# JackWoo0831/Yolov7-tracker

Measured on AMD Instinct MI355X. Metric: end-to-end fps (detect+track) YOLOv7-w6@1280 ByteTrack, higher is better.
Workload: dtype f16

## Files before the change

### yolov7-tracker_amd/csrc/y7t_conv_common.h

```cpp
#pragma once
#include "y7t_det.h"
#include <type_traits>

typedef _Float16 half_t;
typedef __attribute__((ext_vector_type(8))) _Float16 half8;
typedef __attribute__((ext_vector_type(4))) _Float16 half4;
typedef __attribute__((ext_vector_type(16))) float floatx16;

#define GLOBAL_AS __attribute__((address_space(1)))
#define LDS_AS __attribute__((address_space(3)))

template <int ACT>
__device__ __forceinline__ float act_t(float v) {
    if (ACT == Y7T_ACT_SILU) return v * __builtin_amdgcn_rcpf(1.0f + __builtin_amdgcn_exp2f(-1.44269504088896f * v));
    if (ACT == Y7T_ACT_LEAKY) return v > 0.f ? v : 0.1f * v;
    return v;
}

template <typename F>
__device__ __forceinline__ void act_dispatch(int act, F&& body) {
    if (act == Y7T_ACT_SILU) body(std::integral_constant<int, Y7T_ACT_SILU>{});
    else if (act == Y7T_ACT_LEAKY) body(std::integral_constant<int, Y7T_ACT_LEAKY>{});
    else body(std::integral_constant<int, Y7T_ACT_NONE>{});
}

__device__ __forceinline__ float act_fn(float v, int act) {
    if (act == Y7T_ACT_SILU) return v * __builtin_amdgcn_rcpf(1.0f + __builtin_amdgcn_exp2f(-1.44269504088896f * v));
    if (act == Y7T_ACT_LEAKY) return v > 0.f ? v : 0.1f * v;
    return v;
}
```

### yolov7-tracker_amd/csrc/y7t_conv_patch.hip

```cpp
#include "y7t_common.h"
#include "y7t_conv_common.h"
#include <stdlib.h>

namespace {

constexpr unsigned kOOB = 0xFF000000u;

template <int TW, int TH, int BN>
struct PatchCfg {
    static constexpr int PIXB = 80;
    static constexpr bool FLAT = (TW == 0);
    static constexpr int PW = TH;
    static constexpr int NPOS = 256 + 2 * PW + 2;
    static constexpr int RP = FLAT ? PW * PIXB : (TW == 16) ? 1536 : (TW + 2) * PIXB;
    static constexpr int PATCH_DMA = FLAT ? (NPOS * PIXB + 1023) / 1024 : ((TH + 2) * RP + 1023) / 1024;
    static constexpr int NPX = (PATCH_DMA + 1) / 2;
    static constexpr int PATCH_BYTES = PATCH_DMA * 1024;
    static constexpr int PPT = (NPX + 6) / 7;
    static constexpr int WROWB = 64;
    static constexpr int W_DMA = BN * WROWB / 1024;
    static constexpr int NWX = W_DMA / 2;
    static constexpr int W_BYTES = W_DMA * 1024;
    static constexpr int NWS = 3;
    static constexpr int W_OFF = 0, P_OFF = NWS * W_BYTES;
    static constexpr int LDS_LOOP = P_OFF + 2 * PATCH_BYTES;
    static constexpr int OROW = BN * 2 + 16;
    static constexpr int LDS_EPI = 256 * OROW;
    static constexpr int BIAS_OFF = LDS_LOOP > LDS_EPI + 1024 ? LDS_LOOP : LDS_EPI + 1024;
    static constexpr int LDS = BIAS_OFF + BN * 4;
    static constexpr int WN = BN / 64, WM = 4 / WN;
    static constexpr int TM = 8 / WM;
    static constexpr int RPT = (TW == 16) ? 2 : 1;
    static constexpr int JOFF = FLAT ? 32 * PIXB : RPT * RP;
};

#define Y7T_PATCH_ISSUE_DMAS() \
            { \
                constexpr bool live = !(ABL & 1); \
                if (wrole) { \
                    const int un = u + 3; \
                    const int ccn = (un / 9), tn = un % 9; \
                    const int cn = c0 + ccn; \
                    if (ABL & 16) issue_w(u % 3, 0, 0, 0, true); \
                    else issue_w(u % 3, ccn == 2 ? cbase + s_pair : cbase + ccn * s_odd, tn / 3, tn % 3, cn < nc32 && live); \
                } else if (t < 7) { \
                _Pragma("unroll") \
                    for (int q = 0; q < C::PPT; ++q) \
                        if (t * C::PPT + q < C::NPX) issue_patch_piece(cc ^ 1, c + 1, t * C::PPT + q, c + 1 < nc32 && live && !(ABL & 32)); \
                } \
            }
template <int TW, int TH, int BN, int ABL>
__global__ void __launch_bounds__(256, 2) k_conv3x3_patch(const Y7TConvArgs p) {
#if defined(__HIP_DEVICE_COMPILE__)
    using C = PatchCfg<TW, TH, BN>;
    static_assert(C::FLAT || TW * TH == 256, "256 output pixels per workgroup");
    constexpr int PIXB = C::PIXB, RP = C::RP, TM = C::TM, RPT = C::RPT;
    constexpr bool FLAT = C::FLAT;
    extern __shared__ __attribute__((aligned(16))) char smem[];
    const int tid = threadIdx.x, lane = tid & 63, wave = __builtin_amdgcn_readfirstlane(tid >> 6);
    const int wn = (C::WN == 2) ? (wave >> 1) : 0, wm = (C::WN == 2) ? (wave & 1) : wave;
    const int l31 = lane & 31, hi32 = lane >> 5;

    int bid = blockIdx.x;
    if (p.xcd_swizzle) {
        const int nwg = gridDim.x, q = nwg >> 3, r = nwg & 7, xcd = bid & 7, idx = bid >> 3;
        bid = (xcd < r ? xcd * (q + 1) : r * (q + 1) + (xcd - r) * q) + idx;
    }
    const int n_tiles_n = p.Cout_pad / BN;
    const int tile_n = bid % n_tiles_n;
    int pt = bid / n_tiles_n;
    int b = 0, h0 = 0, w0 = 0;
    const int g0 = pt * 256;
    const int img_pos = (p.H + 2) * C::PW, strip = p.B * img_pos;
    if (!FLAT) {
        constexpr int TWd = FLAT ? 1 : TW;
        const int tiles_x = (p.W + TWd - 1) / TWd, tiles_y = (p.H + TH - 1) / TH;
        const int txi = pt % tiles_x; pt /= tiles_x;
        const int tyi = pt % tiles_y;
        b = pt / tiles_y; h0 = tyi * TH; w0 = txi * TWd;
    }
    const int n0 = tile_n * BN;

    const __amdgpu_buffer_rsrc_t xr = __builtin_amdgcn_make_buffer_rsrc((void*)p.in, 0, p.in_bytes, 0x00020000);
    const __amdgpu_buffer_rsrc_t wr = __builtin_amdgcn_make_buffer_rsrc((void*)p.w, 0, p.w_bytes, 0x00020000);

    const bool wrole = wave < 2;
    constexpr int NOFF = C::NPX > C::NWX ? C::NPX : C::NWX;
    unsigned off[NOFF];
#pragma unroll
    for (int i = 0; i < NOFF; ++i) {
        unsigned v = kOOB;
        if (wrole) {
            if (i < C::NWX) {
                const int byte = (wave * C::NWX + i) * 1024 + lane * 16;
                const int row = byte >> 6, slot = (byte >> 4) & 3;
                if (p.korder == 2) v = (unsigned)(tile_n * (p.K_pad >> 5) * C::W_BYTES + byte);
                else v = (unsigned)(((n0 + row) * p.K_pad + ((slot ^ ((row >> 2) & 3)) << 3)) * 2);
            }
        } else if (i < C::NPX) {
            int I = (wave - 2) + 2 * i;
            if (I >= C::PATCH_DMA) I = C::PATCH_DMA - 1;
            const int byte = I * 1024 + lane * 16;
            if (FLAT) {
                const int q = byte / PIXB, cs = (byte - q * PIXB) >> 4;
                const int g = g0 - C::PW - 1 + q;
                if (cs < 4 && q < C::NPOS && g >= 0 && g < strip) {
                    const int bb = g / img_pos, rem = g - bb * img_pos;
                    const int yy = rem / C::PW, xx = rem - yy * C::PW;
                    if (yy >= 1 && yy <= p.H && xx >= 1 && xx <= p.W)
                        v = (unsigned)(((((bb * p.H + yy - 1) * p.W + xx - 1) * p.ldin + p.cin_off) + cs * 8) * 2);
                }
            } else {
            const int r = byte / RP, rb = byte - r * RP;
            const int x = rb / PIXB, cs = (rb - x * PIXB) >> 4;
            const int gy = h0 + r - 1, gx = w0 + x - 1;
            const bool ok = r < TH + 2 && x < TW + 2 && cs < 4 && (unsigned)gy < (unsigned)p.H && (unsigned)gx < (unsigned)p.W;
            if (ok) v = (unsigned)(((((b * p.H + gy) * p.W + gx) * p.ldin + p.cin_off) + cs * 8) * 2);
            }
        }
        off[i] = v;
    }

    const int wsw = (l31 >> 2) & 3;
    const char* wlane0 = smem + C::W_OFF + (wn * 64 + l31) * C::WROWB + (((0 + hi32) ^ wsw) << 4);
    const char* wlane1 = smem + C::W_OFF + (wn * 64 + l31) * C::WROWB + (((2 + hi32) ^ wsw) << 4);
    const char* plane = FLAT ? smem + C::P_OFF + (wm * TM * 32 + l31) * PIXB + hi32 * 16
                             : smem + C::P_OFF + (wm * TM * RPT + (TW == 16 ? (l31 >> 4) : 0)) * RP + (TW == 16 ? (l31 & 15) : l31) * PIXB + hi32 * 16;

    const int nc32 = p.Cin >> 5;
    const int s_kh = p.korder == 2 ? 3 * C::W_BYTES : p.korder ? (p.Cin >> 6) * 3 * 128 : 3 * p.Cin * 2;
    const int s_kw = p.korder == 2 ? C::W_BYTES : p.korder ? 128 : p.Cin * 2;
    const int s_odd = p.korder == 2 ? 9 * C::W_BYTES : 64;
    const int s_pair = p.korder == 2 ? 18 * C::W_BYTES : p.korder ? 3 * 128 : 128;
    int cbase = 0;
    auto issue_w = [&](int slot, int coff, int kh, int kw, bool real) {
        const int so = kh * s_kh + kw * s_kw + coff;
#pragma unroll
        for (int i = 0; i < C::NWX; ++i)
            __builtin_amdgcn_raw_ptr_buffer_load_lds(wr, (LDS_AS void*)(smem + C::W_OFF + slot * C::W_BYTES + (wave * C::NWX + i) * 1024), 16,
                                                     real ? off[i] : kOOB, real ? so : 0, 0, 0);
    };
    auto issue_patch_piece = [&](int pb, int c, int i, bool real) {
        const int I = ((wave - 2) + 2 * i < C::PATCH_DMA) ? (wave - 2) + 2 * i : C::PATCH_DMA - 1;
        __builtin_amdgcn_raw_ptr_buffer_load_lds(xr, (LDS_AS void*)(smem + C::P_OFF + pb * C::PATCH_BYTES + I * 1024), 16,
                                                 real ? off[i] : kOOB, c << 6, 0, 0);
    };

    floatx16 acc[2][TM];
#pragma unroll
    for (int i = 0; i < 2; ++i)
#pragma unroll
        for (int j = 0; j < TM; ++j)
#pragma unroll
            for (int e = 0; e < 16; ++e) acc[i][j][e] = 0.f;

    if (tid < BN) ((float*)(smem + C::BIAS_OFF))[tid] = p.bias[n0 + tid];
    if (wrole) {
        issue_w(0, 0, 0, 0, true);
        issue_w(1, 0, 0, 1, true);
        issue_w(2, 0, 0, 2, true);
    } else {
#pragma unroll
        for (int i = 0; i < C::NPX; ++i) issue_patch_piece(0, 0, i, true);
    }

    static_assert(C::PPT * 7 >= C::NPX, "patch pieces fit into taps 0..6");
    static_assert(C::LDS <= 81920, "two workgroups per CU");
    half8 wf[2][2][2], xf[2][2][TM];
    auto read_frags = [&](int buf, int slot, int pb, int kh, int kw) {
        const char* ws0 = wlane0 + slot * C::W_BYTES;
        const char* ws1 = wlane1 + slot * C::W_BYTES;
        const char* ps = plane + pb * C::PATCH_BYTES + kh * RP + kw * PIXB;
        if (ABL & 4) {
#pragma unroll
            for (int ks = 0; ks < 2; ++ks) {
#pragma unroll
                for (int i = 0; i < 2; ++i) asm volatile("" : "=v"(wf[buf][ks][i]));
#pragma unroll
                for (int j = 0; j < TM; ++j) asm volatile("" : "=v"(xf[buf][ks][j]));
            }
            return;
        }
#pragma unroll
        for (int ks = 0; ks < 2; ++ks) {
#pragma unroll
            for (int i = 0; i < 2; ++i) wf[buf][ks][i] = *(const half8*)((ks ? ws1 : ws0) + i * 32 * C::WROWB);
#pragma unroll
            for (int j = 0; j < TM; ++j) xf[buf][ks][j] = *(const half8*)(ps + j * C::JOFF + ks * 32);
        }
    };
    auto mfma_half = [&](int buf, int ks) {
        if (ABL & 2) {
#pragma unroll
            for (int i = 0; i < 2; ++i) asm volatile("" ::"v"(wf[buf][ks][i]));
#pragma unroll
            for (int j = 0; j < TM; ++j) asm volatile("" ::"v"(xf[buf][ks][j]));
            return;
        }
        __builtin_amdgcn_s_setprio(1);
#pragma unroll
        for (int i = 0; i < 2; ++i)
#pragma unroll
            for (int j = 0; j < TM; ++j) acc[i][j] = __builtin_amdgcn_mfma_f32_32x32x16_f16(wf[buf][ks][i], xf[buf][ks][j], acc[i][j], 0, 0, 0);
        __builtin_amdgcn_s_setprio(0);
    };
    if (wrole) asm volatile("s_waitcnt vmcnt(%0)" ::"n"(2 * C::NWX) : "memory");
    else asm volatile("s_waitcnt vmcnt(0)" ::: "memory");
    __builtin_amdgcn_s_barrier();
    read_frags(0, 0, 0, 0, 0);

    for (int c0 = 0; c0 < nc32; c0 += 2) {
#pragma unroll
        for (int u = 0; u < 18; ++u) {
            const int cc = u / 9, t = u % 9;
            const int c = c0 + cc, cur = u & 1;
            if (ABL == 0) {
                const int un = u + 1, tn = un % 9, kh = tn / 3, kw = tn % 3;
                const char* ps = plane + ((un / 9) & 1) * C::PATCH_BYTES + kh * RP + kw * PIXB;
                const char* ws0 = wlane0 + (un % 3) * C::W_BYTES;
                const char* ws1 = wlane1 + (un % 3) * C::W_BYTES;
                __builtin_amdgcn_s_setprio(1);
#pragma unroll
                for (int q = 0; q < 2 * TM; ++q) {
                    const int i = q / TM, j = q % TM;
                    acc[i][j] = __builtin_amdgcn_mfma_f32_32x32x16_f16(wf[cur][0][i], xf[cur][0][j], acc[i][j], 0, 0, 0);
                    if (t < 8) xf[cur ^ 1][q / TM][q % TM] = *(const half8*)(ps + (q % TM) * C::JOFF + (q / TM) * 32);
                    __builtin_amdgcn_sched_barrier(0);
                }
                __builtin_amdgcn_s_setprio(0);
                if (t < 8) asm volatile("s_waitcnt lgkmcnt(%0)" ::"n"(2 * TM) : "memory");
                else asm volatile("s_waitcnt lgkmcnt(0)" ::: "memory");
                if (wrole) asm volatile("s_waitcnt vmcnt(%0)" ::"n"(C::NWX) : "memory");
                else if (t == 8) asm volatile("s_waitcnt vmcnt(0)" ::: "memory");
                __builtin_amdgcn_s_barrier();
                Y7T_PATCH_ISSUE_DMAS()
                __builtin_amdgcn_sched_barrier(0);
                __builtin_amdgcn_s_setprio(1);
#pragma unroll
                for (int q = 0; q < 2 * TM; ++q) {
                    const int i = q / TM, j = q % TM;
                    acc[i][j] = __builtin_amdgcn_mfma_f32_32x32x16_f16(wf[cur][1][i], xf[cur][1][j], acc[i][j], 0, 0, 0);
                    if (q < 4) wf[cur ^ 1][q >> 1][q & 1] = *(const half8*)(((q >> 1) ? ws1 : ws0) + (q & 1) * 32 * C::WROWB);
                    if (t == 8) xf[cur ^ 1][q / TM][q % TM] = *(const half8*)(ps + (q % TM) * C::JOFF + (q / TM) * 32);
                    __builtin_amdgcn_sched_barrier(0);
                }
                __builtin_amdgcn_s_setprio(0);
                continue;
            }
            mfma_half(cur, 0);
            asm volatile("s_waitcnt lgkmcnt(0)" ::: "memory");
            if (wrole) asm volatile("s_waitcnt vmcnt(%0)" ::"n"(C::NWX) : "memory");
            else if (t == 8) asm volatile("s_waitcnt vmcnt(0)" ::: "memory");
            __builtin_amdgcn_s_barrier();
            if (!(ABL & 512)) Y7T_PATCH_ISSUE_DMAS()
            {
                const int un = u + 1, tn = un % 9;
                read_frags(cur ^ 1, un % 3, (un / 9) & 1, tn / 3, tn % 3);
            }
            mfma_half(cur, 1);
            if (ABL & 512) Y7T_PATCH_ISSUE_DMAS()
        }
        cbase += s_pair;
    }

    if (ABL & 8) {
#pragma unroll
        for (int i = 0; i < 2; ++i)
#pragma unroll
            for (int j = 0; j < TM; ++j) asm volatile("" ::"v"(acc[i][j]));
        return;
    }
    constexpr int OROW = C::OROW;
    const float* lbias = (const float*)(smem + C::BIAS_OFF);
    asm volatile("s_waitcnt vmcnt(0)" ::: "memory");
    __syncthreads();
    typedef __attribute__((ext_vector_type(4))) float float4v;
    act_dispatch(p.act, [&](auto act_c) {
    constexpr int ACT = decltype(act_c)::value;
#pragma unroll
    for (int j = 0; j < TM; ++j) {
        const int pix = (wm * TM + j) * 32 + l31;
#pragma unroll
        for (int i = 0; i < 2; ++i) {
            const int nl = wn * 64 + i * 32;
#pragma unroll
            for (int gp = 0; gp < 2; ++gp) {
                unsigned w[2][2];
#pragma unroll
                for (int gg = 0; gg < 2; ++gg) {
                    const int g = gp * 2 + gg;
                    const int n = n0 + nl + 8 * g + 4 * hi32;
                    float v[4];
                    const float4v bv = *(const float4v*)(lbias + (n - n0));
#pragma unroll
                    for (int e = 0; e < 4; ++e) v[e] = act_t<ACT>(acc[i][j][g * 4 + e] + bv[e]);
                    typedef __attribute__((ext_vector_type(2))) _Float16 half2v;
                    half2v h0 = {(half_t)v[0], (half_t)v[1]}, h1 = {(half_t)v[2], (half_t)v[3]};
                    w[gg][0] = __builtin_bit_cast(unsigned, h0);
                    w[gg][1] = __builtin_bit_cast(unsigned, h1);
                }
                auto r0 = __builtin_amdgcn_permlane32_swap(w[0][0], w[1][0], false, false);
                auto r1 = __builtin_amdgcn_permlane32_swap(w[0][1], w[1][1], false, false);
                typedef __attribute__((ext_vector_type(4))) unsigned uint4v;
                uint4v pk = {r0[0], r1[0], r0[1], r1[1]};
                *(uint4v*)(smem + pix * OROW + (nl + 8 * (gp * 2 + hi32)) * 2) = pk;
            }
        }
    }
    });
    int* otab = (int*)(smem + C::LDS_EPI);
    if (FLAT) {
        const int g = g0 + tid;
        int o = -1;
        if (g < strip) {
            const int bb = g / img_pos, rem = g - bb * img_pos;
            const int yy = rem / C::PW, xx = rem - yy * C::PW;
            if (yy >= 1 && yy <= p.H && xx >= 1 && xx <= p.W) o = (bb * p.H + yy - 1) * p.W + xx - 1;
        }
        otab[tid] = o;
    }
    __syncthreads();
    {
        typedef __attribute__((ext_vector_type(4))) unsigned uint4v;
        constexpr int CPP = BN / 8;
        half_t* outp = (half_t*)p.out;
        constexpr int GRP = CPP < 8 ? CPP : 8;
        static_assert(CPP % GRP == 0, "whole groups");
#pragma unroll 1
        for (int c0 = 0; c0 < CPP; c0 += GRP) {
            uint4v v[GRP];
#pragma unroll
            for (int k = 0; k < GRP; ++k) {
                const int cidx = tid + (c0 + k) * 256, pix = cidx / CPP, ch = cidx - pix * CPP;
                v[k] = *(const uint4v*)(smem + pix * OROW + ch * 16);
            }
            __builtin_amdgcn_sched_barrier(0);
#pragma unroll
            for (int k = 0; k < GRP; ++k) {
                const int cidx = tid + (c0 + k) * 256, pix = cidx / CPP, ch = cidx - pix * CPP;
                const int n = n0 + ch * 8;
                long long opix;
                if (FLAT) opix = otab[pix];
                else {
                    constexpr int TWd = FLAT ? 1 : TW;
                    const int r = pix / TWd, x = pix - r * TWd;
                    const int gy = h0 + r, gx = w0 + x;
                    opix = (gy < p.H && gx < p.W) ? (long long)(b * p.H + gy) * p.W + gx : -1;
                }
                if (opix >= 0 && n < p.Cout) *(uint4v*)(outp + (size_t)opix * p.ldout + p.cout_off + n) = v[k];
            }
        }
    }
#endif
}

template <int TW, int TH, int MT>
__global__ void __launch_bounds__(256, 2) k_conv3x3_patch_mt(const Y7TConvArgs p) {
#if defined(__HIP_DEVICE_COMPILE__)
    constexpr int BN = 64;
    using C = PatchCfg<TW, TH, BN>;
    static_assert(!C::FLAT && TW * TH == 256, "256 output pixels per tile");
    constexpr int PIXB = C::PIXB, RP = C::RP, TM = C::TM, RPT = C::RPT;
    constexpr int NWS = 3, WD = 3;
    constexpr int P_OFF = NWS * C::W_BYTES, BIAS_OFF = P_OFF + 2 * C::PATCH_BYTES;
    extern __shared__ __attribute__((aligned(16))) char smem[];
    const int tid = threadIdx.x, lane = tid & 63, wave = __builtin_amdgcn_readfirstlane(tid >> 6);
    const int wm = wave;
    const int l31 = lane & 31, hi32 = lane >> 5;
    int bid = blockIdx.x;
    if (p.xcd_swizzle) {
        const int nwg = gridDim.x, q = nwg >> 3, r = nwg & 7, xcd = bid & 7, idx = bid >> 3;
        bid = (xcd < r ? xcd * (q + 1) : r * (q + 1) + (xcd - r) * q) + idx;
    }
    const int n_tiles_n = p.Cout_pad / BN;
    const int tile_n = bid % n_tiles_n, n0 = tile_n * BN;
    const int tiles_x = (p.W + TW - 1) / TW, tiles_y = (p.H + TH - 1) / TH, ptiles = p.B * tiles_y * tiles_x;
    const int pt_first = (bid / n_tiles_n) * MT;
    const int nt = (ptiles - pt_first) < MT ? (ptiles - pt_first) : MT;

    const __amdgpu_buffer_rsrc_t xr = __builtin_amdgcn_make_buffer_rsrc((void*)p.in, 0, p.in_bytes, 0x00020000);
    const __amdgpu_buffer_rsrc_t wr = __builtin_amdgcn_make_buffer_rsrc((void*)p.w, 0, p.w_bytes, 0x00020000);
    const bool wrole = wave < 2;

    auto patch_off = [&](int pt, unsigned (&o)[C::NPX]) {
        int q = pt;
        const int txi = q % tiles_x; q /= tiles_x;
        const int tyi = q % tiles_y, b = q / tiles_y, h0 = tyi * TH, w0 = txi * TW;
#pragma unroll
        for (int i = 0; i < C::NPX; ++i) {
            int I = (wave - 2) + 2 * i;
            if (I >= C::PATCH_DMA) I = C::PATCH_DMA - 1;
            const int byte = I * 1024 + lane * 16;
            const int r = byte / RP, rb = byte - r * RP;
            const int x = rb / PIXB, cs = (rb - x * PIXB) >> 4;
            const int gy = h0 + r - 1, gx = w0 + x - 1;
            const bool ok = pt < ptiles && r < TH + 2 && x < TW + 2 && cs < 4 && (unsigned)gy < (unsigned)p.H && (unsigned)gx < (unsigned)p.W;
            o[i] = ok ? (unsigned)(((((b * p.H + gy) * p.W + gx) * p.ldin + p.cin_off) + cs * 8) * 2) : kOOB;
        }
    };
    unsigned pc[C::NPX], pn[C::NPX], woff[C::NWX];
#pragma unroll
    for (int i = 0; i < C::NPX; ++i) pc[i] = pn[i] = kOOB;
#pragma unroll
    for (int i = 0; i < C::NWX; ++i) woff[i] = kOOB;
    if (wrole) {
#pragma unroll
        for (int i = 0; i < C::NWX; ++i) {
            const int byte = (wave * C::NWX + i) * 1024 + lane * 16;
            const int row = byte >> 6, slot = (byte >> 4) & 3;
            woff[i] = p.korder == 2 ? (unsigned)(tile_n * (p.K_pad >> 5) * C::W_BYTES + byte)
                                    : (unsigned)(((n0 + row) * p.K_pad + ((slot ^ ((row >> 2) & 3)) << 3)) * 2);
        }
    } else {
        patch_off(pt_first, pc);
        patch_off(pt_first + 1, pn);
    }
    const int wsw = (l31 >> 2) & 3;
    const char* wlane0 = smem + C::W_OFF + l31 * C::WROWB + (((0 + hi32) ^ wsw) << 4);
    const char* wlane1 = smem + C::W_OFF + l31 * C::WROWB + (((2 + hi32) ^ wsw) << 4);
    const char* plane = smem + P_OFF + (wm * TM * RPT + (TW == 16 ? (l31 >> 4) : 0)) * RP + (TW == 16 ? (l31 & 15) : l31) * PIXB + hi32 * 16;

    const int nc32 = p.Cin >> 5, total = nt * nc32;
    const int s_kh = p.korder == 2 ? 3 * C::W_BYTES : p.korder ? (p.Cin >> 6) * 3 * 128 : 3 * p.Cin * 2;
    const int s_kw = p.korder == 2 ? C::W_BYTES : p.korder ? 128 : p.Cin * 2;
    auto chunk_off = [&](int c) -> int {
// ... 88 lines not shown
        }
        ct += 2;
        if (ct == nc32) {
            int q = pt_first + tcur;
            const int txi = q % tiles_x; q /= tiles_x;
            const int tyi = q % tiles_y, b = q / tiles_y, h0 = tyi * TH, w0 = txi * TW;
            act_dispatch(p.act, [&](auto act_c) {
            constexpr int ACT = decltype(act_c)::value;
            typedef __attribute__((ext_vector_type(4))) float float4v;
#pragma unroll
            for (int j = 0; j < TM; ++j) {
                const int pix = (wm * TM + j) * 32 + l31;
                const int r = pix / TW, x = pix - r * TW;
                const int gy = h0 + r, gx = w0 + x;
                const bool okp = gy < p.H && gx < p.W;
                half_t* orow = outp + ((size_t)(b * p.H + gy) * p.W + gx) * p.ldout + p.cout_off + n0;
#pragma unroll
                for (int i = 0; i < 2; ++i) {
#pragma unroll
                    for (int gp = 0; gp < 2; ++gp) {
                        unsigned w[2][2];
#pragma unroll
                        for (int gg = 0; gg < 2; ++gg) {
                            const int g = gp * 2 + gg;
                            const int nl = i * 32 + 8 * g + 4 * hi32;
                            float v[4];
                            const float4v bv = *(const float4v*)(lbias + nl);
#pragma unroll
                            for (int e = 0; e < 4; ++e) v[e] = act_t<ACT>(acc[i][j][g * 4 + e] + bv[e]);
                            typedef __attribute__((ext_vector_type(2))) _Float16 half2v;
                            half2v h0v = {(half_t)v[0], (half_t)v[1]}, h1v = {(half_t)v[2], (half_t)v[3]};
                            w[gg][0] = __builtin_bit_cast(unsigned, h0v);
                            w[gg][1] = __builtin_bit_cast(unsigned, h1v);
                        }
                        auto r0 = __builtin_amdgcn_permlane32_swap(w[0][0], w[1][0], false, false);
                        auto r1 = __builtin_amdgcn_permlane32_swap(w[0][1], w[1][1], false, false);
                        typedef __attribute__((ext_vector_type(4))) unsigned uint4v;
                        const uint4v pk = {r0[0], r1[0], r0[1], r1[1]};
                        const int nn = i * 32 + 8 * (gp * 2 + hi32);
                        if (okp && n0 + nn < p.Cout) *(uint4v*)(orow + nn) = pk;
                    }
#pragma unroll
                    for (int e = 0; e < 16; ++e) acc[i][j][e] = 0.f;
                }
            }
            });
            ct = 0;
            ++tcur;
            if (!wrole) {
#pragma unroll
                for (int i = 0; i < C::NPX; ++i) pc[i] = pn[i];
                patch_off(pt_first + tcur + 1, pn);
            }
        }
    }
#endif
}

template <int TW, int TH, int MT>
int launch_patch_mt(const Y7TConvArgs& a, hipStream_t s) {
    using C0 = PatchCfg<TW, TH, 64>;
    constexpr int lds = 3 * C0::W_BYTES + 2 * C0::PATCH_BYTES + 64 * 4;
    static_assert(lds <= 81920, "two workgroups per CU");
    static Y7TOncePerDevice attr;
    if (int e_ = y7t_once_per_device(attr, [&]() -> int {
        Y7T_HIP_CHECK(hipFuncSetAttribute((const void*)k_conv3x3_patch_mt<TW, TH, MT>, hipFuncAttributeMaxDynamicSharedMemorySize, lds));
        return 0;
    })) return e_;
    const int ptiles = a.B * ((a.H + TH - 1) / TH) * ((a.W + TW - 1) / TW);
    hipLaunchKernelGGL((k_conv3x3_patch_mt<TW, TH, MT>), dim3(((ptiles + MT - 1) / MT) * (a.Cout_pad / 64)), dim3(256), lds, s, a);
    Y7T_LAUNCH_CHECK();
    y7t_note_kernel("patch_mt<%d,%d,%d>", TW, TH, MT);
    return 0;
}

template <int TW, int TH, int BN, int ABL = 0>
int launch_patch(const Y7TConvArgs& a, hipStream_t s) {
    using C = PatchCfg<TW, TH, BN>;
    static Y7TOncePerDevice attr;
    if (int e_ = y7t_once_per_device(attr, [&]() -> int {
        Y7T_HIP_CHECK(hipFuncSetAttribute((const void*)k_conv3x3_patch<TW, TH, BN, ABL>, hipFuncAttributeMaxDynamicSharedMemorySize, C::LDS));
        return 0;
    })) return e_;
    const int ptiles = C::FLAT ? (a.B * (a.H + 2) * C::PW + 255) / 256 : a.B * ((a.H + TH - 1) / TH) * ((a.W + (C::FLAT ? 1 : TW) - 1) / (C::FLAT ? 1 : TW));
    const int tiles = ptiles * (a.Cout_pad / BN);
    hipLaunchKernelGGL((k_conv3x3_patch<TW, TH, BN, ABL>), dim3(tiles), dim3(256), C::LDS, s, a);
    Y7T_LAUNCH_CHECK();
    if (C::FLAT) y7t_note_kernel("patch_strip<%d,%d>%s", C::PW, BN, ABL == 2048 ? " burst-reads" : "");
    else y7t_note_kernel("patch<%d,%d,%d>%s", TW, TH, BN, ABL == 2048 ? " burst-reads" : "");
    return 0;
}

}

int y7t_conv_patch_try(const Y7TConvArgs& a, hipStream_t s) {
    static int mode = -1;
    if (mode < 0) mode = y7t_exp_switch("Y7T_CONV_PATCH", 1);
    const bool eligible = a.KH == 3 && a.KW == 3 && a.stride == 1 && a.pad == 1 && a.Cin % 64 == 0 && !a.out_f32 && !(a.Cout & 7) && !(a.ldout & 7) &&
                          !(a.cout_off & 7) && a.Ho == a.H && a.Wo == a.W && a.in_bytes <= kOOB - (1u << 24) && a.w_bytes <= kOOB - (1u << 24);
    if (a.korder == 2 && (!eligible || !mode)) {
        y7t_set_error("conv: weights are in panel order (korder 2) but the layer cannot run on the patch kernel");
        return Y7T_E_ARG;
    }
    if (!mode || !eligible) return 0;
    auto eff = [&](int tw, int th) {
        const int tx = (a.W + tw - 1) / tw, ty = (a.H + th - 1) / th;
        return (double)(a.W * a.H) / ((double)tx * tw * ty * th);
    };
    const double e16 = eff(16, 16), e32 = eff(32, 8);
    const bool use16 = e16 >= e32;
    const bool wide = a.Cout_pad % 128 == 0 && !a.panel64;
    const double eflat = (a.W == 40 || a.W == 20) ? (double)(a.W * a.H) / ((a.W + 2) * (a.H + 2)) : 0.0;
    if (!a.force_patch && a.korder != 2 && (long long)a.B * a.H * a.W * (a.Cout_pad / (wide ? 128 : 64)) < 256ll * 256) return 0;
    const int abl = Y7T_ABLATE ? a.ablate : 0;
    if (eflat > (use16 ? e16 : e32) && eflat >= 0.8 && (!abl || abl == 2048)) {
        int rcf;
#if Y7T_ABLATE
        if (abl == 2048) {
            if (a.W == 40) rcf = wide ? launch_patch<0, 42, 128, 2048>(a, s) : launch_patch<0, 42, 64, 2048>(a, s);
            else rcf = wide ? launch_patch<0, 22, 128, 2048>(a, s) : launch_patch<0, 22, 64, 2048>(a, s);
        } else
#endif
        if (a.W == 40) rcf = wide ? launch_patch<0, 42, 128>(a, s) : launch_patch<0, 42, 64>(a, s);
        else rcf = wide ? launch_patch<0, 22, 128>(a, s) : launch_patch<0, 22, 64>(a, s);
        return rcf ? rcf : 1;
    }
    if (!a.force_patch && a.korder != 2 && (use16 ? e16 : e32) < 0.8) return 0;
    int rc;
#if Y7T_ABLATE
    if (abl == 2048) {
        if (use16) rc = wide ? launch_patch<16, 16, 128, 2048>(a, s) : launch_patch<16, 16, 64, 2048>(a, s);
        else rc = wide ? launch_patch<32, 8, 128, 2048>(a, s) : launch_patch<32, 8, 64, 2048>(a, s);
        return rc ? rc : 1;
    }
    if (abl && use16 && wide) {
        switch (abl) {
        case 1: return launch_patch<16, 16, 128, 1>(a, s) ? -1 : 1;
        case 2: return launch_patch<16, 16, 128, 2>(a, s) ? -1 : 1;
        case 4: return launch_patch<16, 16, 128, 4>(a, s) ? -1 : 1;
        case 8: return launch_patch<16, 16, 128, 8>(a, s) ? -1 : 1;
        case 15: return launch_patch<16, 16, 128, 15>(a, s) ? -1 : 1;
        case 16: return launch_patch<16, 16, 128, 16>(a, s) ? -1 : 1;
        case 32: return launch_patch<16, 16, 128, 32>(a, s) ? -1 : 1;
        case 48: return launch_patch<16, 16, 128, 48>(a, s) ? -1 : 1;
        default: break;
        }
    }
#endif
    static int mt = -1;
    if (mt < 0) mt = y7t_exp_switch("Y7T_CONV_PATCH_MT", 1);
    const int ptiles = a.B * ((a.H + (use16 ? 15 : 7)) / (use16 ? 16 : 8)) * ((a.W + (use16 ? 15 : 31)) / (use16 ? 16 : 32));
    if (!wide && mt && !abl && (ptiles * (a.Cout_pad / 64) >= 4 * 2048 || a.force_patch)) {
        rc = use16 ? launch_patch_mt<16, 16, 4>(a, s) : launch_patch_mt<32, 8, 4>(a, s);
        return rc ? rc : 1;
    }
    if (use16) rc = wide ? launch_patch<16, 16, 128>(a, s) : launch_patch<16, 16, 64>(a, s);
    else rc = wide ? launch_patch<32, 8, 128>(a, s) : launch_patch<32, 8, 64>(a, s);
    return rc ? rc : 1;
}
```

### yolov7-tracker_amd/detector/graph.py

```python
import math

import os

import numpy as np

from .. import _lib


def make_divisible(x, divisor):
    return math.ceil(x / divisor) * divisor


class Node:
    __slots__ = ("idx", "kind", "src", "c", "k", "s", "p", "act", "wkey", "layer", "extra", "h", "w", "home", "coff", "ld", "virt_up", "virtual")

    def __init__(self, kind, src, c, k=1, s=1, p=0, act=0, wkey=None, layer=-1, extra=None):
        self.kind, self.src, self.c, self.k, self.s, self.p, self.act, self.wkey, self.layer, self.extra = kind, list(src), c, k, s, p, act, wkey, layer, extra
        self.idx = -1
        self.h = self.w = 0
        self.home, self.coff, self.ld = None, 0, 0
        self.virt_up, self.virtual = None, False


def _act_code(a):
# ... 61 lines not shown
        elif m in ("nn.Upsample", "Upsample"):
            if args[0] not in (None, "None") or args[1] != 2 or args[2] != "nearest":
                raise NotImplementedError("Upsample%r" % (args,))
            out, c2 = add(Node("up", src, cin[0], layer=i)), cin[0]
        elif m == "Shortcut":
            if len(src) != 2 or cin[0] != cin[1]:
                raise NotImplementedError("Shortcut of %d tensors with %r channels" % (len(src), cin))
            out, c2 = add(Node("add", src, cin[0], layer=i)), cin[0]
        elif m == "DownC":
            c2 = make_divisible(args[0] * gw, 8)
            k = args[2] if len(args) > 2 else 2
            key = "model.%d." % i
            cv1 = add(Node("conv", src, cin[0], 1, 1, 0, 1, key + "cv1", i))
            cv2 = add(Node("conv", [cv1], c2 // 2, 3, k, 1, 1, key + "cv2", i))
            mp = add(Node("pool", src, cin[0], k, k, 0, layer=i))
            cv3 = add(Node("conv", [mp], c2 // 2, 1, 1, 0, 1, key + "cv3", i))
            out = add(Node("concat", [cv2, cv3], c2 // 2 * 2, layer=i))
            c2 = c2 // 2 * 2
        elif m == "SPPCSPC":
            c2 = make_divisible(args[0] * gw, 8)
            c_ = int(2 * c2 * 0.5)
            key = "model.%d." % i
            cv1 = add(Node("conv", src, c_, 1, 1, 0, 1, key + "cv1", i))
            cv3 = add(Node("conv", [cv1], c_, 3, 1, 1, 1, key + "cv3", i))
            cv4 = add(Node("conv", [cv3], c_, 1, 1, 0, 1, key + "cv4", i))
            p5 = add(Node("pool", [cv4], c_, 5, 1, 2, layer=i))
            p9 = add(Node("pool", [p5], c_, 5, 1, 2, layer=i))
            p13 = add(Node("pool", [p9], c_, 5, 1, 2, layer=i))
            cat1 = add(Node("concat", [cv4, p5, p9, p13], 4 * c_, layer=i))
            cv5 = add(Node("conv", [cat1], c_, 1, 1, 0, 1, key + "cv5", i))
            cv6 = add(Node("conv", [cv5], c_, 3, 1, 1, 1, key + "cv6", i))
            cv2 = add(Node("conv", src, c_, 1, 1, 0, 1, key + "cv2", i))
            cat2 = add(Node("concat", [cv6, cv2], 2 * c_, layer=i))
            out = add(Node("conv", [cat2], c2, 1, 1, 0, 1, key + "cv7", i))
        elif m in ("Detect", "IDetect", "IAuxDetect"):
            nl = len(anchors)
            out = add(Node("detect", src[:nl], no, layer=i, extra={"kind": m, "nl": nl, "na": na, "no": nc + 5, "cin": cin[:nl]}))
            c2 = no
        else:
            raise NotImplementedError("module %s (layer %d) is outside the yolov7 family's hot path" % (m, i))
        layer_out.append(out)
        chs.append(c2)
    return nodes, layer_out


OP_DTYPE = np.dtype([("type", "<i4"), ("in_buf", "<i4"), ("in_ld", "<i4"), ("in_coff", "<i4"), ("H", "<i4"), ("W", "<i4"), ("Cin", "<i4"),
                     ("out_buf", "<i4"), ("out_ld", "<i4"), ("out_coff", "<i4"), ("out_f32", "<i4"), ("Ho", "<i4"), ("Wo", "<i4"),
                     ("Cout", "<i4"), ("Cout_pad", "<i4"), ("KH", "<i4"), ("KW", "<i4"), ("stride", "<i4"), ("pad", "<i4"), ("K", "<i4"),
                     ("K_pad", "<i4"), ("act", "<i4"), ("korder", "<i4"), ("detect_level", "<i4"), ("w_off", "<i8"), ("bias_off", "<i8"),
                     ("up_buf", "<i4"), ("up_ld", "<i4"), ("up_coff", "<i4"), ("up_c0", "<i4"), ("up_C", "<i4"), ("pad0", "<i4")], align=False)
assert OP_DTYPE.itemsize == 136


def _rup(x, m):
    return (x + m - 1) // m * m


class Plan:
    """result of `lower`: ops (structured array), buffer table, weight layout, head description"""


def patch_panel_rows(H, W, cout, B):
    cout_pad = -(-cout // 64) * 64
    if cout_pad % 128:
        return 64
    below = int(_lib.switch("Y7T_CONV_PATCH_PANEL64_BELOW", "512"))
    return 64 if B * H * W // 256 * (cout_pad // 128) < below else 128


PATCH_MIN_PIX = 100 * 256
PATCH_MIN_PIX_SHALLOW = 50 * 256


def patch_eligible(H, W, cin, cout, k, s, p, out_ld, out_coff, out_f32, B=1 << 20):
    cout_pad = -(-cout // 64) * 64
    bn = patch_panel_rows(H, W, cout, B)
    if B * H * W * (cout_pad // bn) < int(_lib.switch("Y7T_CONV_PATCH_MIN_PIX", str(PATCH_MIN_PIX_SHALLOW if cin <= 128 else PATCH_MIN_PIX))):
        return False
    if _lib.switch("Y7T_CONV_PATCH", "1") == "0" or _lib.switch("Y7T_CONV_VARIANT", "0") != "0":
        return False
    if not (k == 3 and s == 1 and p == 1 and cin % 64 == 0 and not out_f32 and cout % 8 == 0 and out_ld % 8 == 0 and out_coff % 8 == 0):
        return False
    eff = lambda tw, th: (W * H) / float(-(-W // tw) * tw * -(-H // th) * th)
    eflat = (W * H) / float((W + 2) * (H + 2)) if W in (20, 40) else 0.0
    return max(eff(16, 16), eff(32, 8), eflat) >= 0.8


def patch_s2_eligible(cin, cout, k, s, p, out_ld, out_coff, out_f32, M_out=1 << 30):
    mode = _lib.switch("Y7T_CONV_PATCH_S2", "auto")
    if mode == "0" or _lib.switch("Y7T_CONV_VARIANT", "0") != "0":
        return False
    cout_pad = -(-cout // 64) * 64
    can = (k == 3 and s == 2 and p == 1 and cin % 64 == 0 and cout_pad % 128 == 0 and not out_f32 and cout % 8 == 0 and out_ld % 8 == 0
           and out_coff % 8 == 0)
    if mode == "1":
        return can and cout_pad >= int(_lib.switch("Y7T_CONV_PATCH_S2_MIN_COUT", "128"))
    return can and cout_pad % 256 == 0 and cin >= 128 and M_out >= 50000 and _lib.switch("Y7T_CONV_PATCH_S2_BN", "") != "128"


def ws_eligible(H, W, cin, cout, k, s, p, out_ld, out_coff, out_f32, in_ld, in_coff, B=1 << 20):
    if _lib.switch("Y7T_CONV_WS", "1") == "0" or _lib.switch("Y7T_CONV_VARIANT", "0") != "0":
        return False
    tiles = B * -(-H // 16) * -(-W // 16)
    return (k == 3 and s == 1 and p == 1 and cin == 64 and cout == 64 and H % 16 == 0 and W % 16 == 0 and not out_f32 and out_ld % 8 == 0 and out_coff % 8 == 0 and in_ld % 8 == 0
            and in_coff % 8 == 0 and tiles >= int(_lib.switch("Y7T_CONV_WS_MIN_TILES", "1024")))


def ws_s2_eligible(H, W, cin, cout, k, s, p, out_ld, out_coff, out_f32, in_ld, in_coff, B=1 << 20):
    if _lib.switch("Y7T_CONV_WS_S2", "1") == "0" or _lib.switch("Y7T_CONV_VARIANT", "0") != "0":
        return False
    Ho, Wo = H // 2, W // 2
    return (k == 3 and s == 2 and p == 1 and cin == 64 and cout == 128 and H % 2 == 0 and W % 2 == 0 and Ho % 2 == 0 and Wo % 32 == 0 and not out_f32
            and out_ld % 8 == 0 and out_coff % 8 == 0 and in_ld % 8 == 0 and in_coff % 8 == 0 and B * (Ho // 2) * (Wo // 32) >= int(_lib.switch("Y7T_CONV_WS_MIN_TILES", "1024")))


def p8_eligible(H, W, cin, cout, k, s, out_ld, out_coff, out_f32, in_ld, in_coff, B=1 << 20, up=None, detect=False):
    mode = _lib.switch("Y7T_CONV_P8", "1")
    if mode == "0" or _lib.switch("Y7T_CONV_VARIANT", "0") != "0" or detect:
        return False
    tiles = -(-(B * H * W) // 256) * (cout // 256 if cout % 256 == 0 else 0)
    ok = (k == 1 and s == 1 and cin % 64 == 0 and cout % 256 == 0 and not out_f32 and out_ld % 8 == 0 and out_coff % 8 == 0 and in_ld % 8 == 0 and in_coff % 8 == 0
          and tiles >= int(_lib.switch("Y7T_CONV_P8_MIN_TILES", "230")))
    if mode != "all" and _lib.switch("Y7T_CONV_P8_MIN_TILES", None) is None:
        fill = tiles / float(max(1, -(-tiles // 256)) * 256)
        ok = ok and (cin >= 1024 or (cin >= 512 and tiles >= 3000) or tiles >= 1500 or (cin >= 512 and fill >= 0.9))
    if up is not None:
        ok = ok and up[0] % 64 == 0 and up[1] % 64 == 0 and H % 2 == 0 and W % 2 == 0
    return bool(ok)


WS128_DEFAULT = "1"


def ws128_eligible(H, W, cin, cout, k, s, p, out_ld, out_coff, out_f32, in_ld, in_coff, B=1 << 20):
    if _lib.switch("Y7T_CONV_WS128", WS128_DEFAULT) != "1" or _lib.switch("Y7T_CONV_VARIANT", "0") != "0":
        return False
    tiles = B * (H // 4) * (W // 16)
    return (k == 3 and s == 1 and p == 1 and cin == 128 and cout % 128 == 0 and cout <= 512 and H % 4 == 0 and W % 16 == 0 and not out_f32 and out_ld % 8 == 0
            and out_coff % 8 == 0 and in_ld % 8 == 0 and in_coff % 8 == 0 and tiles >= int(_lib.switch("Y7T_CONV_WS_MIN_TILES", "1024")))


WS128_S2_DEFAULT = "1"


def ws128_s2_eligible(H, W, cin, cout, k, s, p, out_ld, out_coff, out_f32, in_ld, in_coff, B=1 << 20):
    if _lib.switch("Y7T_CONV_WS128_S2", WS128_S2_DEFAULT) != "1" or _lib.switch("Y7T_CONV_WS128", WS128_DEFAULT) != "1" or _lib.switch("Y7T_CONV_VARIANT", "0") != "0":
        return False
    Ho, Wo = H // 2, W // 2
    return (k == 3 and s == 2 and p == 1 and cin == 128 and cout % 128 == 0 and cout <= 512 and H % 2 == 0 and W % 2 == 0 and Ho % 2 == 0 and Wo % 16 == 0 and not out_f32
            and out_ld % 8 == 0 and out_coff % 8 == 0 and in_ld % 8 == 0 and in_coff % 8 == 0 and B * (Ho // 2) * (Wo // 16) >= int(_lib.switch("Y7T_CONV_WS_MIN_TILES", "1024")))


def lower(nodes, H, W, max_batch=1):
    det = next(n for n in nodes if n.kind == "detect")
    live = set()
    stack = list(det.src)
    while stack:
        i = stack.pop()
        if i in live:
            continue
        live.add(i)
        stack.extend(nodes[i].src)
    for n in nodes:
        if n.kind == "input":
            n.h, n.w = H, W
            continue
        if n.kind == "detect":
# ... 274 lines not shown
```

Before: 2507.

## Drop padded border positions from flat 3x3 patch conv using LDS zero masking

The flat (row-strip) patch convolution for 20- and 40-wide feature maps used to index a virtually padded (W+2)x(H+2) grid, which wasted work on border output positions. Now it indexes only real pixels and handles out-of-image taps per lane by redirecting LDS reads to a small zeroed region, based on precomputed edge masks. This also removes the output pixel lookup table and the divisions in offset setup. The cost is extra per-lane select logic in the inner fragment loads and a slightly larger LDS footprint.

```diff
diff --git a/yolov7-tracker_amd/csrc/y7t_conv_common.h b/yolov7-tracker_amd/csrc/y7t_conv_common.h
--- a/yolov7-tracker_amd/csrc/y7t_conv_common.h
+++ b/yolov7-tracker_amd/csrc/y7t_conv_common.h
@@ -9,6 +9,11 @@
 
 #define GLOBAL_AS __attribute__((address_space(1)))
 #define LDS_AS __attribute__((address_space(3)))
+
+typedef bool y7t_mask_t;
+__device__ __forceinline__ y7t_mask_t y7t_lane_mask(bool c) { return c; }
+__device__ __forceinline__ const half8* y7t_lds_select(const char* a, const char* z, y7t_mask_t m) { return (const half8*)(m ? z : a); }
+__device__ __forceinline__ const half8* y7t_lds_select2(const char* a, const char* z, y7t_mask_t m0, y7t_mask_t m1) { return (const half8*)((m0 | m1) ? z : a); }
 
 template <int ACT>
 __device__ __forceinline__ float act_t(float v) {
diff --git a/yolov7-tracker_amd/csrc/y7t_conv_patch.hip b/yolov7-tracker_amd/csrc/y7t_conv_patch.hip
--- a/yolov7-tracker_amd/csrc/y7t_conv_patch.hip
+++ b/yolov7-tracker_amd/csrc/y7t_conv_patch.hip
@@ -27,7 +27,10 @@
     static constexpr int OROW = BN * 2 + 16;
     static constexpr int LDS_EPI = 256 * OROW;
     static constexpr int BIAS_OFF = LDS_LOOP > LDS_EPI + 1024 ? LDS_LOOP : LDS_EPI + 1024;
-    static constexpr int LDS = BIAS_OFF + BN * 4;
+    static constexpr int ZERO_OFF = BIAS_OFF + BN * 4;
+    static constexpr int ZERO_BYTES = FLAT ? 240 + 240 + 32 + 16 + 48 : 0;
+    static constexpr int LDS = ZERO_OFF + ZERO_BYTES;
+    static_assert(ZERO_OFF % 256 == 0 && P_OFF % 256 == 0 && PATCH_BYTES % 256 == 0, "slot arithmetic of the zero region");
     static constexpr int WN = BN / 64, WM = 4 / WN;
     static constexpr int TM = 8 / WM;
     static constexpr int RPT = (TW == 16) ? 2 : 1;
@@ -71,7 +74,7 @@
     int pt = bid / n_tiles_n;
     int b = 0, h0 = 0, w0 = 0;
     const int g0 = pt * 256;
-    const int img_pos = (p.H + 2) * C::PW, strip = p.B * img_pos;
+    const int npix = p.B * p.H * p.W;
     if (!FLAT) {
         constexpr int TWd = FLAT ? 1 : TW;
         const int tiles_x = (p.W + TWd - 1) / TWd, tiles_y = (p.H + TH - 1) / TH;
@@ -104,12 +107,7 @@
             if (FLAT) {
                 const int q = byte / PIXB, cs = (byte - q * PIXB) >> 4;
                 const int g = g0 - C::PW - 1 + q;
-                if (cs < 4 && q < C::NPOS && g >= 0 && g < strip) {
-                    const int bb = g / img_pos, rem = g - bb * img_pos;
-                    const int yy = rem / C::PW, xx = rem - yy * C::PW;
-                    if (yy >= 1 && yy <= p.H && xx >= 1 && xx <= p.W)
-                        v = (unsigned)(((((bb * p.H + yy - 1) * p.W + xx - 1) * p.ldin + p.cin_off) + cs * 8) * 2);
-                }
+                if (cs < 4 && q < C::NPOS && g >= 0 && g < npix) v = ((unsigned)g * (unsigned)p.ldin + (unsigned)(p.cin_off + cs * 8)) * 2u;
             } else {
             const int r = byte / RP, rb = byte - r * RP;
             const int x = rb / PIXB, cs = (rb - x * PIXB) >> 4;
@@ -135,13 +133,20 @@
     int cbase = 0;
     auto issue_w = [&](int slot, int coff, int kh, int kw, bool real) {
         const int so = kh * s_kh + kw * s_kw + coff;
+        int wv = wave;
+        if (FLAT) asm volatile("" : "+s"(wv));
 #pragma unroll
         for (int i = 0; i < C::NWX; ++i)
-            __builtin_amdgcn_raw_ptr_buffer_load_lds(wr, (LDS_AS void*)(smem + C::W_OFF + slot * C::W_BYTES + (wave * C::NWX + i) * 1024), 16,
+            __builtin_amdgcn_raw_ptr_buffer_load_lds(wr, (LDS_AS void*)(smem + C::W_OFF + slot * C::W_BYTES + (wv * C::NWX + i) * 1024), 16,
                                                      real ? off[i] : kOOB, real ? so : 0, 0, 0);
     };
     auto issue_patch_piece = [&](int pb, int c, int i, bool real) {
-        const int I = ((wave - 2) + 2 * i < C::PATCH_DMA) ? (wave - 2) + 2 * i : C::PATCH_DMA - 1;
+        int wv = wave - 2;
+        if (FLAT) {
+            asm volatile("" : "+s"(wv));
+            wv &= 1;
+        }
+        const int I = (wv + 2 * i < C::PATCH_DMA) ? wv + 2 * i : C::PATCH_DMA - 1;
         __builtin_amdgcn_raw_ptr_buffer_load_lds(xr, (LDS_AS void*)(smem + C::P_OFF + pb * C::PATCH_BYTES + I * 1024), 16,
                                                  real ? off[i] : kOOB, c << 6, 0, 0);
     };
@@ -164,13 +169,55 @@
         for (int i = 0; i < C::NPX; ++i) issue_patch_piece(0, 0, i, true);
     }
 
+    typedef __attribute__((ext_vector_type(4))) unsigned zero4v;
+    y7t_mask_t mx0[TM] = {}, mxw[TM] = {}, my0[TM] = {}, myh[TM] = {};
+    const int zlane = C::ZERO_OFF + (((5 * l31 + hi32) & 15) << 4);
+    if (FLAT) {
+        if (tid * 16 < C::ZERO_BYTES) *(zero4v*)(smem + C::ZERO_OFF + tid * 16) = zero4v{0u, 0u, 0u, 0u};
+#pragma unroll
+        for (int j = 0; j < TM; ++j) {
+            const int g = g0 + (wm * TM + j) * 32 + l31;
+            const int r = g / C::PW, x = g - r * C::PW, y = r % p.H;
+            mx0[j] = y7t_lane_mask(x == 0);
+            mxw[j] = y7t_lane_mask(x == C::PW - 1);
+            my0[j] = y7t_lane_mask(y == 0);
+            myh[j] = y7t_lane_mask(y == p.H - 1);
+        }
+    }
+    auto patch_frag = [&](const char* ps, const char* zs, int kh, int kw, int j, int ks) -> half8 {
+        if (FLAT && (kh != 1 || kw != 1)) {
+            const char* a = ps + j * C::JOFF;
+            y7t_mask_t my = 0, mx = 0;
+            if (kh == 0) my = my0[j];
+            if (kh == 2) my = myh[j];
+            if (kw == 0) mx = mx0[j];
+            if (kw == 2) mx = mxw[j];
+            if (kh != 1 && kw != 1) return y7t_lds_select2(a, zs, my, mx)[ks * 2];
+            return y7t_lds_select(a, zs, kh != 1 ? my : mx)[ks * 2];
+        }
+        return *(const half8*)(ps + j * C::JOFF + ks * 32);
+    };
+    auto step_plane = [&]() -> const char* {
+        if (!FLAT) return plane;
+        int pl = C::P_OFF + (wm * TM * 32 + l31) * PIXB + hi32 * 16;
+        asm volatile("" : "+v"(pl));
+        return smem + pl;
+    };
+    auto step_zero = [&](int kh, int kw) -> const char* {
+        if (!FLAT) return smem;
+        int zl = zlane;
+        asm volatile("" : "+v"(zl));
+        return smem + zl + (((5 * (kh * C::PW + kw)) & 15) << 4);
+    };
+
     static_assert(C::PPT * 7 >= C::NPX, "patch pieces fit into taps 0..6");
     static_assert(C::LDS <= 81920, "two workgroups per CU");
     half8 wf[2][2][2], xf[2][2][TM];
     auto read_frags = [&](int buf, int slot, int pb, int kh, int kw) {
         const char* ws0 = wlane0 + slot * C::W_BYTES;
         const char* ws1 = wlane1 + slot * C::W_BYTES;
-        const char* ps = plane + pb * C::PATCH_BYTES + kh * RP + kw * PIXB;
+        const char* ps = step_plane() + pb * C::PATCH_BYTES + kh * RP + kw * PIXB;
+        const char* zs = step_zero(kh, kw);
         if (ABL & 4) {
 #pragma unroll
             for (int ks = 0; ks < 2; ++ks) {
@@ -186,7 +233,7 @@
 #pragma unroll
             for (int i = 0; i < 2; ++i) wf[buf][ks][i] = *(const half8*)((ks ? ws1 : ws0) + i * 32 * C::WROWB);
 #pragma unroll
-            for (int j = 0; j < TM; ++j) xf[buf][ks][j] = *(const half8*)(ps + j * C::JOFF + ks * 32);
+            for (int j = 0; j < TM; ++j) xf[buf][ks][j] = patch_frag(ps, zs, kh, kw, j, ks);
         }
     };
     auto mfma_half = [&](int buf, int ks) {
@@ -206,6 +253,7 @@
     };
     if (wrole) asm volatile("s_waitcnt vmcnt(%0)" ::"n"(2 * C::NWX) : "memory");
     else asm volatile("s_waitcnt vmcnt(0)" ::: "memory");
+    if (FLAT) asm volatile("s_waitcnt lgkmcnt(0)" ::: "memory");
     __builtin_amdgcn_s_barrier();
     read_frags(0, 0, 0, 0, 0);
 
@@ -216,7 +264,8 @@
             const int c = c0 + cc, cur = u & 1;
             if (ABL == 0) {
                 const int un = u + 1, tn = un % 9, kh = tn / 3, kw = tn % 3;
-                const char* ps = plane + ((un / 9) & 1) * C::PATCH_BYTES + kh * RP + kw * PIXB;
+                const char* ps = step_plane() + ((un / 9) & 1) * C::PATCH_BYTES + kh * RP + kw * PIXB;
+                const char* zs = step_zero(kh, kw);
                 const char* ws0 = wlane0 + (un % 3) * C::W_BYTES;
                 const char* ws1 = wlane1 + (un % 3) * C::W_BYTES;
                 __builtin_amdgcn_s_setprio(1);
@@ -224,7 +273,7 @@
                 for (int q = 0; q < 2 * TM; ++q) {
                     const int i = q / TM, j = q % TM;
                     acc[i][j] = __builtin_amdgcn_mfma_f32_32x32x16_f16(wf[cur][0][i], xf[cur][0][j], acc[i][j], 0, 0, 0);
-                    if (t < 8) xf[cur ^ 1][q / TM][q % TM] = *(const half8*)(ps + (q % TM) * C::JOFF + (q / TM) * 32);
+                    if (t < 8) xf[cur ^ 1][q / TM][q % TM] = patch_frag(ps, zs, kh, kw, q % TM, q / TM);
                     __builtin_amdgcn_sched_barrier(0);
                 }
                 __builtin_amdgcn_s_setprio(0);
@@ -241,7 +290,7 @@
                     const int i = q / TM, j = q % TM;
                     acc[i][j] = __builtin_amdgcn_mfma_f32_32x32x16_f16(wf[cur][1][i], xf[cur][1][j], acc[i][j], 0, 0, 0);
                     if (q < 4) wf[cur ^ 1][q >> 1][q & 1] = *(const half8*)(((q >> 1) ? ws1 : ws0) + (q & 1) * 32 * C::WROWB);
-                    if (t == 8) xf[cur ^ 1][q / TM][q % TM] = *(const half8*)(ps + (q % TM) * C::JOFF + (q / TM) * 32);
+                    if (t == 8) xf[cur ^ 1][q / TM][q % TM] = patch_frag(ps, zs, kh, kw, q % TM, q / TM);
                     __builtin_amdgcn_sched_barrier(0);
                 }
                 __builtin_amdgcn_s_setprio(0);
@@ -308,17 +357,6 @@
         }
     }
     });
-    int* otab = (int*)(smem + C::LDS_EPI);
-    if (FLAT) {
-        const int g = g0 + tid;
-        int o = -1;
-        if (g < strip) {
-            const int bb = g / img_pos, rem = g - bb * img_pos;
-            const int yy = rem / C::PW, xx = rem - yy * C::PW;
-            if (yy >= 1 && yy <= p.H && xx >= 1 && xx <= p.W) o = (bb * p.H + yy - 1) * p.W + xx - 1;
-        }
-        otab[tid] = o;
-    }
     __syncthreads();
     {
         typedef __attribute__((ext_vector_type(4))) unsigned uint4v;
@@ -340,7 +378,7 @@
                 const int cidx = tid + (c0 + k) * 256, pix = cidx / CPP, ch = cidx - pix * CPP;
                 const int n = n0 + ch * 8;
                 long long opix;
-                if (FLAT) opix = otab[pix];
+                if (FLAT) opix = g0 + pix < npix ? g0 + pix : -1;
                 else {
                     constexpr int TWd = FLAT ? 1 : TW;
                     const int r = pix / TWd, x = pix - r * TWd;
@@ -595,7 +633,7 @@
         Y7T_HIP_CHECK(hipFuncSetAttribute((const void*)k_conv3x3_patch<TW, TH, BN, ABL>, hipFuncAttributeMaxDynamicSharedMemorySize, C::LDS));
         return 0;
     })) return e_;
-    const int ptiles = C::FLAT ? (a.B * (a.H + 2) * C::PW + 255) / 256 : a.B * ((a.H + TH - 1) / TH) * ((a.W + (C::FLAT ? 1 : TW) - 1) / (C::FLAT ? 1 : TW));
+    const int ptiles = C::FLAT ? (a.B * a.H * a.W + 255) / 256 : a.B * ((a.H + TH - 1) / TH) * ((a.W + (C::FLAT ? 1 : TW) - 1) / (C::FLAT ? 1 : TW));
     const int tiles = ptiles * (a.Cout_pad / BN);
     hipLaunchKernelGGL((k_conv3x3_patch<TW, TH, BN, ABL>), dim3(tiles), dim3(256), C::LDS, s, a);
     Y7T_LAUNCH_CHECK();
@@ -623,19 +661,19 @@
     const double e16 = eff(16, 16), e32 = eff(32, 8);
     const bool use16 = e16 >= e32;
     const bool wide = a.Cout_pad % 128 == 0 && !a.panel64;
-    const double eflat = (a.W == 40 || a.W == 20) ? (double)(a.W * a.H) / ((a.W + 2) * (a.H + 2)) : 0.0;
+    const double eflat = (a.W == 40 || a.W == 20) ? 1.0 : 0.0;
     if (!a.force_patch && a.korder != 2 && (long long)a.B * a.H * a.W * (a.Cout_pad / (wide ? 128 : 64)) < 256ll * 256) return 0;
     const int abl = Y7T_ABLATE ? a.ablate : 0;
     if (eflat > (use16 ? e16 : e32) && eflat >= 0.8 && (!abl || abl == 2048)) {
         int rcf;
 #if Y7T_ABLATE
         if (abl == 2048) {
-            if (a.W == 40) rcf = wide ? launch_patch<0, 42, 128, 2048>(a, s) : launch_patch<0, 42, 64, 2048>(a, s);
-            else rcf = wide ? launch_patch<0, 22, 128, 2048>(a, s) : launch_patch<0, 22, 64, 2048>(a, s);
+            if (a.W == 40) rcf = wide ? launch_patch<0, 40, 128, 2048>(a, s) : launch_patch<0, 40, 64, 2048>(a, s);
+            else rcf = wide ? launch_patch<0, 20, 128, 2048>(a, s) : launch_patch<0, 20, 64, 2048>(a, s);
         } else
 #endif
-        if (a.W == 40) rcf = wide ? launch_patch<0, 42, 128>(a, s) : launch_patch<0, 42, 64>(a, s);
-        else rcf = wide ? launch_patch<0, 22, 128>(a, s) : launch_patch<0, 22, 64>(a, s);
+        if (a.W == 40) rcf = wide ? launch_patch<0, 40, 128>(a, s) : launch_patch<0, 40, 64>(a, s);
+        else rcf = wide ? launch_patch<0, 20, 128>(a, s) : launch_patch<0, 20, 64>(a, s);
         return rcf ? rcf : 1;
     }
     if (!a.force_patch && a.korder != 2 && (use16 ? e16 : e32) < 0.8) return 0;
diff --git a/yolov7-tracker_amd/detector/graph.py b/yolov7-tracker_amd/detector/graph.py
--- a/yolov7-tracker_amd/detector/graph.py
+++ b/yolov7-tracker_amd/detector/graph.py
@@ -167,7 +167,7 @@
     if not (k == 3 and s == 1 and p == 1 and cin % 64 == 0 and not out_f32 and cout % 8 == 0 and out_ld % 8 == 0 and out_coff % 8 == 0):
         return False
     eff = lambda tw, th: (W * H) / float(-(-W // tw) * tw * -(-H // th) * th)
-    eflat = (W * H) / float((W + 2) * (H + 2)) if W in (20, 40) else 0.0
+    eflat = 1.0 if W in (20, 40) else 0.0
     return max(eff(16, 16), eff(32, 8), eflat) >= 0.8
 
 
```

Measured after the change: 2547 (median of 6 runs). +1.6%, better.
